# skyepurchase/MeatModeler

Measured on AMD Instinct MI355X. Metric: descriptor-match pairs/sec + BA residuals/sec, 500×1080p frames, 1/2/4/8 GPU, higher is better.
Workload: dtype u8/int32 (match), f64 (BA); 1 GPU; 500 frames 1920x1080, 4000 ORB kpts/frame, BF Hamming 2-NN + ratio, track linking, 2-view DLT, full BA (TRF, Schur, f64 MFMA Cholesky); frames=500, height=1080, width=1920, nfeatures=4000, parallelism=pairs/points x1

## Files before the change

### meatmodeler_amd/csrc/schur.hip

```cpp
#include "ba_eval.h"
#include "chol_init.h"

namespace {

constexpr int SR_WIN = 256;

__global__ __launch_bounds__(256) void point_inverse_kernel(int P, const double *__restrict__ Cd,
                                                            double *__restrict__ Cinv) {
    int p = blockIdx.x * 256 + threadIdx.x;
    if (p >= P) return;
    const double *c = Cd + (size_t)p * 6;
    const double a = c[0], b = c[1], d = c[2], e = c[3], f = c[4], g = c[5];
    const double m00 = e * g - f * f, m01 = d * f - b * g, m02 = b * f - d * e;
    const double det = a * m00 + b * m01 + d * m02;
    const double id = 1.0 / det;
    double *o = Cinv + (size_t)p * 6;
    o[0] = m00 * id;
    o[1] = m01 * id;
    o[2] = m02 * id;
    o[3] = (a * g - d * d) * id;
    o[4] = (b * d - a * f) * id;
    o[5] = (a * e - b * b) * id;
}

__global__ __launch_bounds__(256) void schur_rows_kernel(mm_ba_problem pb, const double *__restrict__ cams,
                                                         const double *__restrict__ pts, const double *__restrict__ Bd,
                                                         const double *__restrict__ Cinv, const double *__restrict__ gc,
                                                         const double *__restrict__ gp, double *__restrict__ S,
                                                         double *__restrict__ v) {
    __shared__ double acc[6][SR_WIN * 6];
    __shared__ double Ks[9];
    __shared__ double cs[6];
    __shared__ double sm[4];
    const int i = blockIdx.x;
    const int w0 = blockIdx.y * SR_WIN;
    const int wn = min(SR_WIN, pb.F - w0);
    const size_t n = (size_t)pb.F * 6;
    for (int e = threadIdx.x; e < 6 * SR_WIN * 6; e += 256) (&acc[0][0])[e] = 0.0;
    if (threadIdx.x < 9) Ks[threadIdx.x] = pb.K[threadIdx.x];
    if (threadIdx.x < 6) cs[threadIdx.x] = cams[(size_t)i * 6 + threadIdx.x];
    __syncthreads();
    double vg[6] = {0, 0, 0, 0, 0, 0};
    for (int e = pb.cam_ptr[i] + threadIdx.x; e < pb.cam_ptr[i + 1]; e += 256) {
        const int o = pb.cam_obs[e];
        const int p = pb.pi[o];
        const double *Xp = pts + (size_t)p * 3;
        Proj pr;
        ba_eval<true, true>(cs, Xp, Ks, pb.obs[2 * (size_t)o], pb.obs[2 * (size_t)o + 1], pr);
        const double *ci = Cinv + (size_t)p * 6;
        const double q00 = ci[0], q01 = ci[1], q02 = ci[2], q11 = ci[3], q12 = ci[4], q22 = ci[5];
        double Y[6][3];
#pragma unroll
        for (int a = 0; a < 6; ++a) {
            const double e0 = pr.Jc[0][a] * pr.Jp[0][0] + pr.Jc[1][a] * pr.Jp[1][0];
            const double e1 = pr.Jc[0][a] * pr.Jp[0][1] + pr.Jc[1][a] * pr.Jp[1][1];
            const double e2 = pr.Jc[0][a] * pr.Jp[0][2] + pr.Jc[1][a] * pr.Jp[1][2];
            Y[a][0] = e0 * q00 + e1 * q01 + e2 * q02;
            Y[a][1] = e0 * q01 + e1 * q11 + e2 * q12;
            Y[a][2] = e0 * q02 + e1 * q12 + e2 * q22;
        }
        if (blockIdx.y == 0) {
            const double g0 = gp[(size_t)p * 3], g1 = gp[(size_t)p * 3 + 1], g2 = gp[(size_t)p * 3 + 2];
#pragma unroll
            for (int a = 0; a < 6; ++a) vg[a] += Y[a][0] * g0 + Y[a][1] * g1 + Y[a][2] * g2;
        }
        for (int e2i = pb.pt_ptr[p]; e2i < pb.pt_ptr[p + 1]; ++e2i) {
            const int o2 = pb.pt_obs[e2i];
            const int f2 = pb.fi[o2];
            if (f2 < w0 || f2 >= w0 + wn) continue;
            Proj p2;
            ba_eval<true, true>(cams + (size_t)f2 * 6, Xp, Ks, pb.obs[2 * (size_t)o2], pb.obs[2 * (size_t)o2 + 1], p2);
            double *dst = &acc[0][(f2 - w0) * 6];
#pragma unroll
            for (int b = 0; b < 6; ++b) {
                const double e0 = p2.Jc[0][b] * p2.Jp[0][0] + p2.Jc[1][b] * p2.Jp[1][0];
                const double e1 = p2.Jc[0][b] * p2.Jp[0][1] + p2.Jc[1][b] * p2.Jp[1][1];
                const double e2 = p2.Jc[0][b] * p2.Jp[0][2] + p2.Jc[1][b] * p2.Jp[1][2];
#pragma unroll
                for (int a = 0; a < 6; ++a)
                    atomicAdd(dst + a * (SR_WIN * 6) + b, Y[a][0] * e0 + Y[a][1] * e1 + Y[a][2] * e2);
            }
        }
    }
    __syncthreads();
    for (int e = threadIdx.x; e < 6 * wn * 6; e += 256) {
        const int a = e / (wn * 6), c = e % (wn * 6);
        const int col = w0 * 6 + c;
        double val = -acc[a][c];
        if (col / 6 == i) val += Bd[(size_t)i * 36 + a * 6 + (col % 6)];
        S[((size_t)i * 6 + a) * n + col] = val;
    }
    if (blockIdx.y == 0) {
#pragma unroll
        for (int a = 0; a < 6; ++a) {
            const double s = block_sum<256>(vg[a], sm);
            if (threadIdx.x == 0) v[(size_t)i * 6 + a] = gc[(size_t)i * 6 + a] - s;
        }
    }
}

#ifndef MM_SP_WAVES
#define MM_SP_WAVES 1
#endif
constexpr int SP_WAVES = MM_SP_WAVES;
constexpr int MAX_SLABS = 64;
struct SlabSync {
    int32_t *ready;
    int32_t *done;
    int32_t seg_count[MAX_SLABS];
    int cams_per_slab;
};
constexpr int CAMTAB = 11;
__device__ __forceinline__ void write_chunk_desc(const mm_ba_problem &pb, int32_t *__restrict__ desc, int64_t first, int64_t stride) {
    for (int64_t k = first; k < pb.n_chunks; k += stride) {
        const int sidx = pb.chunk_seg[k], seg = pb.seg_ids[sidx];
        const int ci = seg / (pb.cam_span + 1), cdd = seg % (pb.cam_span + 1);
        const int c_first = pb.seg_chunk_ptr[sidx];
        int32_t *o = desc + 8 * k;
        o[0] = ci;
        o[1] = ci - cdd;
        o[2] = pb.chunk_begin[k];
        o[3] = pb.chunk_end[k];
        o[4] = sidx;
        o[5] = c_first;
        o[6] = pb.seg_chunk_ptr[sidx + 1] - c_first;
        o[7] = 0;
    }
}
__global__ __launch_bounds__(64) void cam_table_kernel(int F, const double *__restrict__ cams, double *__restrict__ tab,
                                                       int32_t *__restrict__ seg_done, int64_t n_seg, const double *__restrict__ K_lean,
                                                       mm_ba_problem pb, int32_t *__restrict__ desc) {
    const int f = blockIdx.x * 64 + threadIdx.x;
    for (int64_t k = f; k < n_seg; k += (int64_t)gridDim.x * 64) seg_done[k] = 0;
    if (desc) write_chunk_desc(pb, desc, f, (int64_t)gridDim.x * 64);
    if (f >= F) return;
    const double *c = cams + (size_t)f * 6;
    if (K_lean) {
        cam_table2_row(c, K_lean, tab + (size_t)f * CAMTAB2);
        return;
    }
    const CamCoef k = cam_coef_of(c);
    double *t = tab + (size_t)f * CAMTAB;
    for (int q = 0; q < 6; ++q) t[q] = c[q];
    t[6] = k.c;
    t[7] = k.a;
    t[8] = k.b;
    t[9] = k.a1;
    t[10] = k.b1;
}

__device__ __forceinline__ CamVals cam_vals_from_table(const double *__restrict__ t) {
    CamVals v;
    v.rx = uniform_f64(t[0]);
    v.ry = uniform_f64(t[1]);
    v.rz = uniform_f64(t[2]);
    v.tx = uniform_f64(t[3]);
    v.ty = uniform_f64(t[4]);
    v.tz = uniform_f64(t[5]);
    v.k.c = uniform_f64(t[6]);
    v.k.a = uniform_f64(t[7]);
    v.k.b = uniform_f64(t[8]);
    v.k.a1 = uniform_f64(t[9]);
    v.k.b1 = uniform_f64(t[10]);
    return v;
}

constexpr int RED_LD = 65;
__device__ __forceinline__ void wave_lds_barrier() {
    __builtin_amdgcn_fence(__ATOMIC_RELEASE, "wavefront");
    __builtin_amdgcn_wave_barrier();
    __builtin_amdgcn_fence(__ATOMIC_ACQUIRE, "wavefront");
}
__device__ __forceinline__ void wave_reduce_42(const double (&acc)[42], double *slab , int lane, double &out0,
                                               double &out1) {
#pragma unroll
    for (int h = 0; h < 2; ++h) {
#pragma unroll
        for (int q = 0; q < 21; ++q) slab[q * RED_LD + lane] = acc[21 * h + q];
        wave_lds_barrier();
        double s = 0.0;
        if (lane < 21) {
            const double *row = slab + lane * RED_LD;
            double s0 = 0.0, s1 = 0.0, s2 = 0.0, s3 = 0.0;
#pragma unroll
            for (int j = 0; j < 64; j += 4) {
                s0 += row[j];
                s1 += row[j + 1];
                s2 += row[j + 2];
                s3 += row[j + 3];
            }
            s = (s0 + s1) + (s2 + s3);
        }
        if (h == 0)
            out0 = s;
        else
            out1 = s;
        wave_lds_barrier();
    }
}

__global__ __launch_bounds__(64 * SP_WAVES, 2) void schur_pairs_ref_kernel(mm_ba_problem pb, const double *__restrict__ camtab,
                                                                    const double *__restrict__ pts,
                                                                    const double *__restrict__ Cinv,
                                                                    const double *__restrict__ gp,
                                                                    double *partial, const double *__restrict__ Bd,
                                                                    const double *__restrict__ gc, double *S, double *v,
                                                                    int32_t *seg_done, SlabSync slabs, unsigned wg_begin,
                                                                    unsigned wg_total) {
    __shared__ double Ks[9];
    __shared__ double red[SP_WAVES][21 * RED_LD];
    if (threadIdx.x < 9) Ks[threadIdx.x] = pb.K[threadIdx.x];
    __syncthreads();
    const int lane = threadIdx.x & 63;
    const unsigned gpos = blockIdx.x + wg_begin;
    const unsigned wg = (gpos & 1) ? wg_total - 1 - (gpos >> 1) : (gpos >> 1);
    const int64_t c = (int64_t)wg * SP_WAVES + (threadIdx.x >> 6);
    if (c >= pb.n_chunks) return;
    const int sidx = __builtin_amdgcn_readfirstlane(pb.chunk_seg[c]);
    const int seg = __builtin_amdgcn_readfirstlane(pb.seg_ids[sidx]);
    const int i = seg / (pb.cam_span + 1), d = seg % (pb.cam_span + 1);
    const int f2 = i - d;
    const CamVals cv_i = cam_vals_from_table(camtab + (size_t)i * CAMTAB), cv_2 = cam_vals_from_table(camtab + (size_t)f2 * CAMTAB);
    double acc[42];
#pragma unroll
    for (int q = 0; q < 42; ++q) acc[q] = 0.0;
    const int e_end = __builtin_amdgcn_readfirstlane(pb.chunk_end[c]);
    const int e_begin = __builtin_amdgcn_readfirstlane(pb.chunk_begin[c]);
    constexpr int MAXT = 4;
    int oi[MAXT], o2i[MAXT], pidx[MAXT];
#pragma unroll
    for (int k = 0; k < MAXT; ++k) {
        const int e = e_begin + lane + 64 * k;
        const bool in = e < e_end;
        oi[k] = in ? pb.pair_o[e] : -1;
        o2i[k] = in ? pb.pair_o2[e] : -1;
        pidx[k] = in ? (pb.pair_p ? pb.pair_p[e] : -2) : -1;
    }
    auto pair_body = [&](int o, int o2, int p) {
        const double *Xp = pts + (size_t)p * 3;
        Proj pr;
        ba_eval_vals<true, true>(cv_i, Xp, Ks, pb.obs[2 * (size_t)o], pb.obs[2 * (size_t)o + 1], pr);
        const double *ci = Cinv + (size_t)p * 6;
        const double q00 = ci[0], q01 = ci[1], q02 = ci[2], q11 = ci[3], q12 = ci[4], q22 = ci[5];
        double Z[2][3];
#pragma unroll
        for (int m = 0; m < 2; ++m) {
            Z[m][0] = pr.Jp[m][0] * q00 + pr.Jp[m][1] * q01 + pr.Jp[m][2] * q02;
            Z[m][1] = pr.Jp[m][0] * q01 + pr.Jp[m][1] * q11 + pr.Jp[m][2] * q12;
            Z[m][2] = pr.Jp[m][0] * q02 + pr.Jp[m][1] * q12 + pr.Jp[m][2] * q22;
        }
        if (o2 == o) {
            const double g0 = gp[(size_t)p * 3], g1 = gp[(size_t)p * 3 + 1], g2 = gp[(size_t)p * 3 + 2];
            const double z0 = Z[0][0] * g0 + Z[0][1] * g1 + Z[0][2] * g2, z1 = Z[1][0] * g0 + Z[1][1] * g1 + Z[1][2] * g2;
#pragma unroll
            for (int a = 0; a < 6; ++a) acc[36 + a] += pr.Jc[0][a] * z0 + pr.Jc[1][a] * z1;
        }
        Proj p2;
        ba_eval_vals<true, true>(cv_2, Xp, Ks, pb.obs[2 * (size_t)o2], pb.obs[2 * (size_t)o2 + 1], p2);
        double M[2][2];
#pragma unroll
        for (int m = 0; m < 2; ++m)
#pragma unroll
            for (int n_ = 0; n_ < 2; ++n_) M[m][n_] = Z[m][0] * p2.Jp[n_][0] + Z[m][1] * p2.Jp[n_][1] + Z[m][2] * p2.Jp[n_][2];
#pragma unroll
        for (int b = 0; b < 6; ++b) {
            const double t0 = M[0][0] * p2.Jc[0][b] + M[0][1] * p2.Jc[1][b], t1 = M[1][0] * p2.Jc[0][b] + M[1][1] * p2.Jc[1][b];
#pragma unroll
            for (int a = 0; a < 6; ++a) acc[a * 6 + b] += pr.Jc[0][a] * t0 + pr.Jc[1][a] * t1;
        }
    };
    const int trips = (e_end - e_begin + 63) / 64;
    for (int k = 0; k < MAXT; ++k) {
        if (k >= trips) break;
        int o = oi[0], o2 = o2i[0], p = pidx[0];
#pragma unroll
        for (int q = 1; q < MAXT; ++q)
            if (q == k) {
                o = oi[q];
                o2 = o2i[q];
                p = pidx[q];
            }
        if (o >= 0) {
            if (p == -2) p = pb.pi[o];
            pair_body(o, o2, p);
        }
    }
    for (int e = e_begin + lane + 64 * MAXT; e < e_end; e += 64) {
        const int o = pb.pair_o[e], o2 = pb.pair_o2[e];
        pair_body(o, o2, pb.pair_p ? pb.pair_p[e] : pb.pi[o]);
    }
    double tot0, tot1;
    wave_reduce_42(acc, red[threadIdx.x >> 6], lane, tot0, tot1);
    const int c_first = pb.seg_chunk_ptr[sidx], n_ch = pb.seg_chunk_ptr[sidx + 1] - c_first;
    const size_t n = (size_t)pb.F * 6;
    bool writer = true;
    if (n_ch > 1) {
        if (lane < 21) {
            __hip_atomic_store(partial + (size_t)c * 42 + lane, tot0, __ATOMIC_RELAXED, __HIP_MEMORY_SCOPE_AGENT);
            __hip_atomic_store(partial + (size_t)c * 42 + 21 + lane, tot1, __ATOMIC_RELAXED, __HIP_MEMORY_SCOPE_AGENT);
        }
        asm volatile("s_waitcnt vmcnt(0)" ::: "memory");
        __builtin_amdgcn_wave_barrier();
        int last = 0;
        if (lane == 0) last = atomicAdd(seg_done + sidx, 1) == n_ch - 1;
        writer = __shfl(last, 0, 64) != 0;
        if (writer && lane < 21) {
            tot0 = 0.0;
            tot1 = 0.0;
            for (int cc = 0; cc < n_ch; ++cc) {
                tot0 += __hip_atomic_load(partial + (size_t)(c_first + cc) * 42 + lane, __ATOMIC_RELAXED, __HIP_MEMORY_SCOPE_AGENT);
                tot1 += __hip_atomic_load(partial + (size_t)(c_first + cc) * 42 + 21 + lane, __ATOMIC_RELAXED, __HIP_MEMORY_SCOPE_AGENT);
            }
        }
    }
    if (!writer) return;
    if (lane < 21) {
#pragma unroll
        for (int h = 0; h < 2; ++h) {
            const int q = 21 * h + lane;
            const double sum = h == 0 ? tot0 : tot1;
            if (q < 36) {
                double val = -sum;
                if (d == 0) val += Bd[(size_t)i * 36 + q];
                __hip_atomic_store(S + ((size_t)i * 6 + q / 6) * n + (size_t)f2 * 6 + q % 6, val, __ATOMIC_RELAXED, __HIP_MEMORY_SCOPE_AGENT);
                if (d != 0)
                    __hip_atomic_store(S + ((size_t)f2 * 6 + q % 6) * n + (size_t)i * 6 + q / 6, val, __ATOMIC_RELAXED, __HIP_MEMORY_SCOPE_AGENT);
            } else if (d == 0) {
                __hip_atomic_store(v + (size_t)i * 6 + (q - 36), gc[(size_t)i * 6 + (q - 36)] - sum, __ATOMIC_RELAXED, __HIP_MEMORY_SCOPE_AGENT);
            }
        }
    }
    if (slabs.ready) {
        asm volatile("s_waitcnt vmcnt(0)" ::: "memory");
        __builtin_amdgcn_wave_barrier();
        if (lane == 0) {
            const int sl = i / slabs.cams_per_slab;
            if (atomicAdd(slabs.done + sl, 1) == slabs.seg_count[sl] - 1)
                __hip_atomic_store(slabs.ready + sl, 1, __ATOMIC_RELEASE, __HIP_MEMORY_SCOPE_AGENT);
        }
    }
}


struct CamPQ {
    double P[9], q[3];
};
__device__ __forceinline__ double fast_rcp(double x) {
    double y = __builtin_amdgcn_rcp(x);
    double e = fma(-x, y, 1.0);
    y = fma(y, e, y);
    e = fma(-x, y, 1.0);
    return fma(y, e, y);
}

struct LeanJ {
    double Jc[2][6];
    double Jp[2][3];
};
__device__ __forceinline__ void lean_eval(const CamPQ &c, const double *__restrict__ Ks, const double *__restrict__ Jr,
                                          double X0, double X1, double X2, LeanJ &o) {
    const double u0 = fma(c.P[0], X0, fma(c.P[1], X1, fma(c.P[2], X2, c.q[0])));
    const double u1 = fma(c.P[3], X0, fma(c.P[4], X1, fma(c.P[5], X2, c.q[1])));
    const double u2 = fma(c.P[6], X0, fma(c.P[7], X1, fma(c.P[8], X2, c.q[2])));
    const double iz = fast_rcp(u2);
    const double p[2] = {u0 * iz, u1 * iz};
#pragma unroll
    for (int m = 0; m < 2; ++m) {
#pragma unroll
        for (int k = 0; k < 3; ++k) {
            o.Jp[m][k] = fma(-p[m], c.P[6 + k], c.P[3 * m + k]) * iz;
            o.Jc[m][3 + k] = fma(-p[m], Ks[6 + k], Ks[3 * m + k]) * iz;
        }
        const double g0 = X1 * o.Jp[m][2] - X2 * o.Jp[m][1];
        const double g1 = X2 * o.Jp[m][0] - X0 * o.Jp[m][2];
        const double g2 = X0 * o.Jp[m][1] - X1 * o.Jp[m][0];
#pragma unroll
        for (int k = 0; k < 3; ++k) o.Jc[m][k] = fma(g0, Jr[k], fma(g1, Jr[3 + k], g2 * Jr[6 + k]));
    }
}

constexpr int SLAB2 = 32;
struct ChunkDesc {
    int32_t i, f2, e_begin, e_end, sidx, c_first, n_ch, pad;
};
template <bool FORCE>
__device__ __forceinline__ CamPQ cam_pq_scalar(const double *__restrict__ t) {
    CamPQ v;
#pragma unroll
    for (int k = 0; k < 9; ++k) v.P[k] = FORCE ? uniform_f64(t[k]) : t[k];
#pragma unroll
    for (int k = 0; k < 3; ++k) v.q[k] = FORCE ? uniform_f64(t[9 + k]) : t[9 + k];
    return v;
}
template <bool FORCE_UNIFORM>
__device__ __forceinline__ void schur_pairs_body(const mm_ba_problem pb, const double *__restrict__ camtab,
                                                                    const ChunkDesc *__restrict__ desc,
                                                                    const double *__restrict__ pts,
                                                                    const double *__restrict__ Cinv,
                                                                    const double *__restrict__ gp,
                                                                    double *partial, const double *__restrict__ Bd,
                                                                    const double *__restrict__ gc, double *S, double *v,
                                                                    int32_t *seg_done, SlabSync slabs, unsigned wg_begin,
                                                                    unsigned wg_total, const unsigned bx) {
    __shared__ double Ks[9];
    __shared__ double red[SP_WAVES][21 * RED_LD];
    __shared__ double jrs[SP_WAVES][SLAB2];
    if (threadIdx.x < 9) Ks[threadIdx.x] = pb.K[threadIdx.x];
    const int lane = threadIdx.x & 63;
    const int wv = __builtin_amdgcn_readfirstlane((int)(threadIdx.x >> 6));
    const unsigned gpos = bx + wg_begin;
    const unsigned wg = (gpos & 1) ? wg_total - 1 - (gpos >> 1) : (gpos >> 1);
    const int64_t c = (int64_t)wg * SP_WAVES + wv;
    const bool live = c < pb.n_chunks;
    ChunkDesc cd = {};
    if (live) cd = desc[c];
    if (FORCE_UNIFORM) {
        cd.i = __builtin_amdgcn_readfirstlane(cd.i);
        cd.f2 = __builtin_amdgcn_readfirstlane(cd.f2);
        cd.e_begin = __builtin_amdgcn_readfirstlane(cd.e_begin);
        cd.e_end = __builtin_amdgcn_readfirstlane(cd.e_end);
        cd.sidx = __builtin_amdgcn_readfirstlane(cd.sidx);
        cd.c_first = __builtin_amdgcn_readfirstlane(cd.c_first);
        cd.n_ch = __builtin_amdgcn_readfirstlane(cd.n_ch);
    }
    const int i = cd.i, f2 = cd.f2, d = cd.i - cd.f2, sidx = cd.sidx;
    const int e_begin = cd.e_begin, e_end = cd.e_end;
    auto point_of = [&](int e) { return pb.pair_p ? pb.pair_p[e] : pb.pi[pb.pair_o[e]]; };
    auto self_of = [&](int e) { return d == 0 && pb.pair_o[e] == pb.pair_o2[e]; };
    int e = e_begin + lane;
    int p_next = -1;
    bool self_next = false;
    if (live) {
        if (e < e_end) {
            p_next = point_of(e);
            self_next = self_of(e);
        }
        if (lane < 9) jrs[wv][lane] = camtab[(size_t)i * CAMTAB2 + 12 + lane];
        else if (lane >= 16 && lane < 25) jrs[wv][lane] = camtab[(size_t)f2 * CAMTAB2 + 12 + lane - 16];
    }
    __syncthreads();
    if (!live) return;
    const CamPQ cp_i = cam_pq_scalar<FORCE_UNIFORM>(camtab + (size_t)i * CAMTAB2), cp_2 = cam_pq_scalar<FORCE_UNIFORM>(camtab + (size_t)f2 * CAMTAB2);
    const double *Jr_i = jrs[wv], *Jr_2 = jrs[wv] + 16;
    double acc[42];
#pragma unroll
    for (int q = 0; q < 42; ++q) acc[q] = 0.0;
    auto load_xc = [&](int p, double (&x)[12]) {
        if (p >= 0) {
            const double *Xp = pts + (size_t)p * 3, *ci = Cinv + (size_t)p * 6;
            x[0] = Xp[0];
            x[1] = Xp[1];
            x[2] = Xp[2];
#pragma unroll
            for (int q = 0; q < 6; ++q) x[3 + q] = ci[q];
            if (d == 0) {
                x[9] = gp[(size_t)p * 3];
                x[10] = gp[(size_t)p * 3 + 1];
                x[11] = gp[(size_t)p * 3 + 2];
            }
        }
    };
    auto pair_body = [&](int p, bool self, const double (&x)[12]) {
        const double X0 = x[0], X1 = x[1], X2 = x[2];
        const double q00 = x[3], q01 = x[4], q02 = x[5], q11 = x[6], q12 = x[7], q22 = x[8];
        LeanJ a;
        lean_eval(cp_i, Ks, Jr_i, X0, X1, X2, a);
        double Z[2][3];
#pragma unroll
        for (int m = 0; m < 2; ++m) {
            Z[m][0] = a.Jp[m][0] * q00 + a.Jp[m][1] * q01 + a.Jp[m][2] * q02;
            Z[m][1] = a.Jp[m][0] * q01 + a.Jp[m][1] * q11 + a.Jp[m][2] * q12;
            Z[m][2] = a.Jp[m][0] * q02 + a.Jp[m][1] * q12 + a.Jp[m][2] * q22;
        }
        double M[2][2], T[2][6];
        if (d == 0) {
            if (self) {
                const double g0 = x[9], g1 = x[10], g2 = x[11];
                const double z0 = Z[0][0] * g0 + Z[0][1] * g1 + Z[0][2] * g2, z1 = Z[1][0] * g0 + Z[1][1] * g1 + Z[1][2] * g2;
#pragma unroll
                for (int q = 0; q < 6; ++q) acc[36 + q] += a.Jc[0][q] * z0 + a.Jc[1][q] * z1;
            }
#pragma unroll
            for (int m = 0; m < 2; ++m)
#pragma unroll
                for (int n_ = 0; n_ < 2; ++n_) M[m][n_] = Z[m][0] * a.Jp[n_][0] + Z[m][1] * a.Jp[n_][1] + Z[m][2] * a.Jp[n_][2];
#pragma unroll
            for (int b = 0; b < 6; ++b) {
                T[0][b] = M[0][0] * a.Jc[0][b] + M[0][1] * a.Jc[1][b];
                T[1][b] = M[1][0] * a.Jc[0][b] + M[1][1] * a.Jc[1][b];
            }
        } else {
            LeanJ b2;
            lean_eval(cp_2, Ks, Jr_2, X0, X1, X2, b2);
#pragma unroll
            for (int m = 0; m < 2; ++m)
#pragma unroll
                for (int n_ = 0; n_ < 2; ++n_) M[m][n_] = Z[m][0] * b2.Jp[n_][0] + Z[m][1] * b2.Jp[n_][1] + Z[m][2] * b2.Jp[n_][2];
#pragma unroll
            for (int b = 0; b < 6; ++b) {
                T[0][b] = M[0][0] * b2.Jc[0][b] + M[0][1] * b2.Jc[1][b];
                T[1][b] = M[1][0] * b2.Jc[0][b] + M[1][1] * b2.Jc[1][b];
            }
        }
#pragma unroll
        for (int q = 0; q < 6; ++q)
#pragma unroll
            for (int b = 0; b < 6; ++b) acc[q * 6 + b] += a.Jc[0][q] * T[0][b] + a.Jc[1][q] * T[1][b];
    };
    double xc[12];
    load_xc(p_next, xc);
    int p_cur = p_next;
    bool self_cur = self_next;
    {
        const int en = e + 64;
        p_next = en < e_end ? point_of(en) : -1;
        self_next = en < e_end && self_of(en);
    }
#pragma clang loop unroll(disable)
    for (; e - lane < e_end; e += 64) {
        double xn[12];
        load_xc(p_next, xn);
        const int p_nn_e = e + 128;
        const int p_nn = p_nn_e < e_end ? point_of(p_nn_e) : -1;
        const bool self_nn = p_nn_e < e_end && self_of(p_nn_e);
        if (p_cur >= 0) pair_body(p_cur, self_cur, xc);
#pragma unroll
        for (int q = 0; q < 12; ++q) xc[q] = xn[q];
        p_cur = p_next;
        self_cur = self_next;
        p_next = p_nn;
        self_next = self_nn;
    }
    double tot0, tot1;
    wave_reduce_42(acc, red[wv], lane, tot0, tot1);
    const int c_first = cd.c_first, n_ch = cd.n_ch;
    const size_t n = (size_t)pb.F * 6;
    bool writer = true;
    if (n_ch > 1) {
        if (lane < 21) {
            __hip_atomic_store(partial + (size_t)c * 42 + lane, tot0, __ATOMIC_RELAXED, __HIP_MEMORY_SCOPE_AGENT);
            __hip_atomic_store(partial + (size_t)c * 42 + 21 + lane, tot1, __ATOMIC_RELAXED, __HIP_MEMORY_SCOPE_AGENT);
        }
        asm volatile("s_waitcnt vmcnt(0)" ::: "memory");
        __builtin_amdgcn_wave_barrier();
        int last = 0;
        if (lane == 0) last = atomicAdd(seg_done + sidx, 1) == n_ch - 1;
        writer = __shfl(last, 0, 64) != 0;
        if (writer && lane < 21) {
            tot0 = 0.0;
            tot1 = 0.0;
            for (int cc = 0; cc < n_ch; ++cc) {
                tot0 += __hip_atomic_load(partial + (size_t)(c_first + cc) * 42 + lane, __ATOMIC_RELAXED, __HIP_MEMORY_SCOPE_AGENT);
                tot1 += __hip_atomic_load(partial + (size_t)(c_first + cc) * 42 + 21 + lane, __ATOMIC_RELAXED, __HIP_MEMORY_SCOPE_AGENT);
            }
        }
    }
    if (!writer) return;
    const bool through = slabs.ready != nullptr;
    if (lane < 21) {
#pragma unroll
        for (int h = 0; h < 2; ++h) {
            const int q = 21 * h + lane;
            const double sum = h == 0 ? tot0 : tot1;
            if (q < 36) {
                double val = -sum;
                if (d == 0) val += Bd[(size_t)i * 36 + q];
                double *dst = S + ((size_t)i * 6 + q / 6) * n + (size_t)f2 * 6 + q % 6;
                double *mir = S + ((size_t)f2 * 6 + q % 6) * n + (size_t)i * 6 + q / 6;
                if (through) {
                    __hip_atomic_store(dst, val, __ATOMIC_RELAXED, __HIP_MEMORY_SCOPE_AGENT);
                    if (d != 0) __hip_atomic_store(mir, val, __ATOMIC_RELAXED, __HIP_MEMORY_SCOPE_AGENT);
                } else {
                    *dst = val;
                    if (d != 0) *mir = val;
                }
            } else if (d == 0) {
                double *dst = v + (size_t)i * 6 + (q - 36);
                const double val = gc[(size_t)i * 6 + (q - 36)] - sum;
                if (through) __hip_atomic_store(dst, val, __ATOMIC_RELAXED, __HIP_MEMORY_SCOPE_AGENT);
                else *dst = val;
            }
        }
    }
    if (slabs.ready) {
        asm volatile("s_waitcnt vmcnt(0)" ::: "memory");
        __builtin_amdgcn_wave_barrier();
        if (lane == 0) {
            const int sl = i / slabs.cams_per_slab;
            if (atomicAdd(slabs.done + sl, 1) == slabs.seg_count[sl] - 1)
                __hip_atomic_store(slabs.ready + sl, 1, __ATOMIC_RELEASE, __HIP_MEMORY_SCOPE_AGENT);
        }
    }
}
template <int OCC>
__global__ __launch_bounds__(64 * SP_WAVES, OCC) void schur_pairs_kernel(mm_ba_problem pb, const double *__restrict__ camtab,
                                                                    const ChunkDesc *__restrict__ desc,
                                                                    const double *__restrict__ pts,
                                                                    const double *__restrict__ Cinv,
                                                                    const double *__restrict__ gp,
                                                                    double *partial, const double *__restrict__ Bd,
                                                                    const double *__restrict__ gc, double *S, double *v,
                                                                    int32_t *seg_done, SlabSync slabs, unsigned wg_begin,
                                                                    unsigned wg_total) {
    schur_pairs_body<false>(pb, camtab, desc, pts, Cinv, gp, partial, Bd, gc, S, v, seg_done, slabs, wg_begin, wg_total, blockIdx.x);
}
__global__ __launch_bounds__(256) void zero_batch_kernel(const mm_batch_prob *__restrict__ tab, const int32_t *__restrict__ list) {
    const mm_batch_prob &bp = tab[list[blockIdx.y]];
    if (blockIdx.x >= bp.g_zero) return;
    double2 *S2 = reinterpret_cast<double2 *>(bp.S);
    const int64_t n2 = bp.nc * bp.nc / 2;
    for (int64_t i = (int64_t)blockIdx.x * 256 + threadIdx.x; i < n2; i += (int64_t)bp.g_zero * 256) S2[i] = make_double2(0.0, 0.0);
}
__global__ __launch_bounds__(64 * SP_WAVES, 2) void schur_pairs_batch_kernel(const mm_batch_prob *__restrict__ tab, const int32_t *__restrict__ list) {
    const mm_batch_prob &bp = tab[list[blockIdx.y]];
    if (blockIdx.x >= bp.g_pairs) return;
    SlabSync none = {};
    schur_pairs_body<true>(bp.pb, bp.schur_camtab, (const ChunkDesc *)bp.schur_desc, bp.x + bp.nc, bp.Cinv, bp.g + bp.nc, bp.schur_partial, bp.Bd,
                     bp.g, bp.S, bp.v, bp.schur_seg_done, none, 0u, bp.g_pairs, blockIdx.x);
}




__global__ void slab_flag_kernel(int32_t *flags, int s) {
    __hip_atomic_store(flags + s, 1, __ATOMIC_RELEASE, __HIP_MEMORY_SCOPE_AGENT);
}

__global__ void schur_diag_fill_kernel(mm_ba_problem pb, const double *__restrict__ Bd, const double *__restrict__ gc,
                                       double *__restrict__ S, double *__restrict__ v) {
    const int i = blockIdx.x;
    if (pb.cam_ptr[i + 1] != pb.cam_ptr[i]) return;
    const size_t n = (size_t)pb.F * 6;
    if (threadIdx.x < 36) S[((size_t)i * 6 + threadIdx.x / 6) * n + (size_t)i * 6 + threadIdx.x % 6] = Bd[(size_t)i * 36 + threadIdx.x];
    if (threadIdx.x < 6) v[(size_t)i * 6 + threadIdx.x] = gc[(size_t)i * 6 + threadIdx.x];
}

struct PrepExtra {
    mm_damp_spec dmp;
    int zero_bwb;
    int chol_init;
    mm_chol_init_args init;
};
__device__ __forceinline__ void schur_prepare_body(mm_ba_problem pb, const double *__restrict__ cams,
                                                            double *__restrict__ Bd, const double *__restrict__ Cd,
                                                            const double *__restrict__ gc, double *__restrict__ Cinv,
                                                            double *__restrict__ S, double *__restrict__ v,
                                                            double *__restrict__ tab, int32_t *__restrict__ seg_done, bool lean,
                                                            int32_t *__restrict__ desc , const unsigned bx, const unsigned gx,
                                                            const PrepExtra *ex = nullptr) {
    const int b = (int)bx, tid = threadIdx.x;
    for (int64_t k = (int64_t)b * 256 + tid; k < pb.n_seg; k += (int64_t)gx * 256) seg_done[k] = 0;
    if (desc) write_chunk_desc(pb, desc, (int64_t)b * 256 + tid, (int64_t)gx * 256);
    const bool fold = ex && ex->dmp.B;
    double reg = 0.0;
    if (fold) {
        if (ex->dmp.gh2) {
            const double r = trf_damping_value(ex->dmp.gh2[0], ex->dmp.d11[0], ex->dmp.Delta);
            reg = fmax(r, ex->dmp.min_damping);
            if (b == 0 && tid == 0) {
                ex->dmp.damp_out[0] = r;
                ex->dmp.damp_out[1] = reg;
            }
        } else {
            reg = ex->dmp.reg[0];
        }
    }
    if (ex && ex->chol_init) mm_chol_init_body(ex->init, bx, gx);
    const size_t n = (size_t)pb.F * 6;
    if (ex && ex->zero_bwb >= 0) {
        const int nblk = (int)((n + 63) / 64);
        for (size_t r = bx; r < n; r += gx) {
            const int bi = (int)(r >> 6);
            const int lo = bi - ex->zero_bwb < 0 ? 0 : bi - ex->zero_bwb, hi = bi + ex->zero_bwb >= nblk ? nblk - 1 : bi + ex->zero_bwb;
            const size_t c0 = (size_t)lo * 64, c1 = (size_t)(hi + 1) * 64 < n ? (size_t)(hi + 1) * 64 : n;
            const size_t d0 = r / 6 * 6;
            for (size_t c = c0 + 2 * (size_t)tid; c < c1; c += 512)
                if (c < d0 || c >= d0 + 6) *reinterpret_cast<double2 *>(S + r * n + c) = double2{0.0, 0.0};
        }
    }
    const int f = b * 256 + tid;
    if (f < pb.F) {
        const double *c = cams + (size_t)f * 6;
        if (lean) {
            cam_table2_row(c, pb.K, tab + (size_t)f * CAMTAB2);
        } else {
            const CamCoef k = cam_coef_of(c);
            double *t = tab + (size_t)f * CAMTAB;
            for (int q = 0; q < 6; ++q) t[q] = c[q];
            t[6] = k.c;
            t[7] = k.a;
            t[8] = k.b;
            t[9] = k.a1;
            t[10] = k.b1;
        }
    }
    if (b < pb.F) {
        const bool empty = pb.cam_ptr[b + 1] == pb.cam_ptr[b];
        if (tid < 36) {
            double bd;
            if (fold) {
                bd = ex->dmp.B[(size_t)b * 36 + tid];
                if (tid % 7 == 0) {
                    const double s = ex->dmp.si[(size_t)b * 6 + tid / 7];
                    bd = fma(s * s, reg, bd);
                }
                Bd[(size_t)b * 36 + tid] = bd;
            } else {
                bd = Bd[(size_t)b * 36 + tid];
            }
            if (empty)
                S[((size_t)b * 6 + tid / 6) * n + (size_t)b * 6 + tid % 6] = bd;
            else if (ex && ex->zero_bwb >= 0)
                S[((size_t)b * 6 + tid / 6) * n + (size_t)b * 6 + tid % 6] = 0.0;
        }
        if (empty && tid < 6) v[(size_t)b * 6 + tid] = gc[(size_t)b * 6 + tid];
    }
    const int p = b * 256 + tid;
    if (p < pb.P) {
        double a, bq, d, e, ff, g;
        if (fold) {
            const double *c = ex->dmp.C + (size_t)p * 6;
            const double *sp = ex->dmp.si + n + (size_t)p * 3;
            a = fma(sp[0] * sp[0], reg, c[0]);
            bq = c[1];
            d = c[2];
            e = fma(sp[1] * sp[1], reg, c[3]);
            ff = c[4];
            g = fma(sp[2] * sp[2], reg, c[5]);
        } else {
            const double *c = Cd + (size_t)p * 6;
            a = c[0], bq = c[1], d = c[2], e = c[3], ff = c[4], g = c[5];
        }
        const double m00 = e * g - ff * ff, m01 = d * ff - bq * g, m02 = bq * ff - d * e;
        const double det = a * m00 + bq * m01 + d * m02;
        const double id = 1.0 / det;
        double *o = Cinv + (size_t)p * 6;
        o[0] = m00 * id;
        o[1] = m01 * id;
        o[2] = m02 * id;
        o[3] = (a * g - d * d) * id;
        o[4] = (bq * d - a * ff) * id;
        o[5] = (a * e - bq * bq) * id;
    }
}
__global__ __launch_bounds__(256) void schur_prepare_kernel(mm_ba_problem pb, const double *__restrict__ cams,
                                                            double *__restrict__ Bd, const double *__restrict__ Cd,
                                                            const double *__restrict__ gc, double *__restrict__ Cinv,
                                                            double *__restrict__ S, double *__restrict__ v,
                                                            double *__restrict__ tab, int32_t *__restrict__ seg_done, bool lean,
                                                            int32_t *__restrict__ desc) {
    schur_prepare_body(pb, cams, Bd, Cd, gc, Cinv, S, v, tab, seg_done, lean, desc, blockIdx.x, gridDim.x);
}
__global__ __launch_bounds__(256) void schur_prepare_damped_kernel(mm_ba_problem pb, const double *__restrict__ cams,
                                                                   double *__restrict__ Bd, const double *__restrict__ gc,
                                                                   double *__restrict__ Cinv, double *__restrict__ S,
                                                                   double *__restrict__ v, double *__restrict__ tab,
                                                                   int32_t *__restrict__ seg_done, int32_t *__restrict__ desc,
                                                                   PrepExtra ex) {
    schur_prepare_body(pb, cams, Bd, nullptr, gc, Cinv, S, v, tab, seg_done, true, desc, blockIdx.x, gridDim.x, &ex);
}
__global__ __launch_bounds__(256) void schur_prepare_batch_kernel(const mm_batch_prob *__restrict__ tab, const int32_t *__restrict__ list) {
    const mm_batch_prob &bp = tab[list[blockIdx.y]];
    if (blockIdx.x >= bp.g_prep) return;
    schur_prepare_body(bp.pb, bp.x, bp.Bd, bp.Cd, bp.g, bp.Cinv, bp.S, bp.v, bp.schur_camtab, bp.schur_seg_done, true, bp.schur_desc,
                       blockIdx.x, bp.g_prep);
}


__global__ __launch_bounds__(256) void pairs_count_kernel(mm_ba_problem pb, int32_t *__restrict__ cnt,
                                                          int32_t *__restrict__ span_out) {
    const int64_t o = (int64_t)blockIdx.x * 256 + threadIdx.x;
    int dmax = 0;
    if (o < pb.O) {
        const int f = pb.fi[o], p = pb.pi[o];
        int c = 0;
        for (int e = pb.pt_ptr[p]; e < pb.pt_ptr[p + 1]; ++e) {
            const int d = f - pb.fi[pb.pt_obs[e]];
            c += d >= 0;
            dmax = max(dmax, d);
        }
        cnt[o] = c;
    }
    for (int off = 32; off > 0; off >>= 1) dmax = max(dmax, __shfl_down(dmax, off, 64));
    if ((threadIdx.x & 63) == 0 && dmax > __hip_atomic_load(span_out, __ATOMIC_RELAXED, __HIP_MEMORY_SCOPE_AGENT)) atomicMax(span_out, dmax);
}

__global__ __launch_bounds__(256) void pairs_emit_kernel(mm_ba_problem pb, const int64_t *__restrict__ offsets, int span,
                                                         int32_t *__restrict__ key, int32_t *__restrict__ po,
                                                         int32_t *__restrict__ po2) {
    const int64_t o = (int64_t)blockIdx.x * 256 + threadIdx.x;
    if (o >= pb.O) return;
    const int f = pb.fi[o], p = pb.pi[o];
    int64_t w = offsets[o];
    for (int e = pb.pt_ptr[p]; e < pb.pt_ptr[p + 1]; ++e) {
        const int o2 = pb.pt_obs[e];
        const int d = f - pb.fi[o2];
        if (d < 0) continue;
        key[w] = f * (span + 1) + d;
        po[w] = (int32_t)o;
        po2[w] = o2;
        ++w;
    }
}

}

extern "C" int mm_ba_pairs_count(mm_ctx *ctx, const mm_ba_problem *pb, int32_t *cnt, int32_t *span_out) {
    if (!ctx) return MM_ERR_ARG;
    if (!pb || !cnt || !span_out || (pb->O > 0 && (!pb->fi || !pb->pi || !pb->pt_ptr || !pb->pt_obs)))
        return mm_fail(ctx, MM_ERR_ARG, "mm_ba_pairs_count: bad argument");
    MM_HIP(ctx, hipMemsetAsync(span_out, 0, sizeof(int32_t), ctx->stream));
    if (pb->O == 0) return MM_OK;
    MM_LAUNCH(ctx, "pairs_count_kernel", pairs_count_kernel, dim3((unsigned)((pb->O + 255) / 256)), dim3(256), 0, *pb, cnt,
              span_out);
    return MM_OK;
}

extern "C" int mm_ba_pairs_emit(mm_ctx *ctx, const mm_ba_problem *pb, const int64_t *offsets, int span, int32_t *key,
                                int32_t *pair_o, int32_t *pair_o2) {
    if (!ctx) return MM_ERR_ARG;
    if (!pb || !offsets || !key || !pair_o || !pair_o2 || span < 0) return mm_fail(ctx, MM_ERR_ARG, "mm_ba_pairs_emit: bad argument");
    if (pb->O == 0) return MM_OK;
    if ((int64_t)pb->F * (span + 1) > 0x7fffffffLL) return mm_fail(ctx, MM_ERR_ARG, "mm_ba_pairs_emit: F * (span + 1) overflows the key");
    MM_LAUNCH(ctx, "pairs_emit_kernel", pairs_emit_kernel, dim3((unsigned)((pb->O + 255) / 256)), dim3(256), 0, *pb, offsets,
              span, key, pair_o, pair_o2);
    return MM_OK;
}

extern "C" size_t mm_ba_schur_workspace_bytes(const mm_ba_problem *pb) {
    if (!pb || pb->n_chunks <= 0) return 0;
    return mm_align_up((size_t)pb->n_chunks * 42 * sizeof(double), 256)  +
           mm_align_up((size_t)pb->n_seg * sizeof(int32_t), 256)  +
           mm_align_up(2 * MAX_SLABS * sizeof(int32_t), 256)  +
           mm_align_up((size_t)pb->F * CAMTAB2 * sizeof(double), 256)  +
// ... 211 lines not shown
```

Measured before the change: 9112 billion descriptor pairs/s (match stage).

## Restructure Schur pair loop into templated software pipeline with clamped indices

Rewrites the per-chunk Schur-complement accumulation loop as a templated routine specialised on diagonal vs off-diagonal blocks and on whether a direct pair-to-point index exists. Index loads are clamped instead of predicated, and the loop rotates a ring of register buffers with a configurable prefetch depth, with an optional second level of index indirection prefetched ahead. The goal is to hide gather latency and remove per-iteration branches and copies. The cost is more register pressure from the extra buffers and more code from the four instantiations. The metric shown is the match stage, which this kernel does not touch.

```diff
diff --git a/meatmodeler_amd/csrc/schur.hip b/meatmodeler_amd/csrc/schur.hip
--- a/meatmodeler_amd/csrc/schur.hip
+++ b/meatmodeler_amd/csrc/schur.hip
@@ -1,5 +1,6 @@
 #include "ba_eval.h"
 #include "chol_init.h"
+#include <type_traits>
 
 namespace {
 
@@ -103,6 +104,11 @@
 #define MM_SP_WAVES 1
 #endif
 constexpr int SP_WAVES = MM_SP_WAVES;
+#ifndef MM_SP_DEPTH
+#define MM_SP_DEPTH 1
+#endif
+constexpr int SP_DEPTH = MM_SP_DEPTH;
+static_assert(SP_DEPTH == 1 || SP_DEPTH == 2, "MM_SP_DEPTH: one or two trips ahead");
 constexpr int MAX_SLABS = 64;
 struct SlabSync {
     int32_t *ready;
@@ -425,15 +431,15 @@
     }
     const int i = cd.i, f2 = cd.f2, d = cd.i - cd.f2, sidx = cd.sidx;
     const int e_begin = cd.e_begin, e_end = cd.e_end;
-    auto point_of = [&](int e) { return pb.pair_p ? pb.pair_p[e] : pb.pi[pb.pair_o[e]]; };
-    auto self_of = [&](int e) { return d == 0 && pb.pair_o[e] == pb.pair_o2[e]; };
-    int e = e_begin + lane;
-    int p_next = -1;
-    bool self_next = false;
+    const int e_last = e_end - 1;
+    const bool any = live && e_end > e_begin;
+    int p0 = 0, o0 = 0, o0b = 0;
     if (live) {
-        if (e < e_end) {
-            p_next = point_of(e);
-            self_next = self_of(e);
+        if (any) {
+            const int ec = min(e_begin + lane, e_last);
+            if (!pb.pair_p || d == 0) o0 = pb.pair_o[ec];
+            if (d == 0) o0b = pb.pair_o2[ec];
+            p0 = pb.pair_p ? pb.pair_p[ec] : pb.pi[o0];
         }
         if (lane < 9) jrs[wv][lane] = camtab[(size_t)i * CAMTAB2 + 12 + lane];
         else if (lane >= 16 && lane < 25) jrs[wv][lane] = camtab[(size_t)f2 * CAMTAB2 + 12 + lane - 16];
@@ -445,91 +451,117 @@
     double acc[42];
 #pragma unroll
     for (int q = 0; q < 42; ++q) acc[q] = 0.0;
-    auto load_xc = [&](int p, double (&x)[12]) {
-        if (p >= 0) {
+    auto run_trips = [&](auto diag_c, auto hasp_c) {
+        constexpr bool DIAG = decltype(diag_c)::value, HAS_P = decltype(hasp_c)::value;
+        constexpr int NX = DIAG ? 12 : 9;
+        constexpr int NB = SP_DEPTH + 1;
+        auto gather = [&](int p, double (&x)[NX]) {
             const double *Xp = pts + (size_t)p * 3, *ci = Cinv + (size_t)p * 6;
             x[0] = Xp[0];
             x[1] = Xp[1];
             x[2] = Xp[2];
 #pragma unroll
             for (int q = 0; q < 6; ++q) x[3 + q] = ci[q];
-            if (d == 0) {
+            if (DIAG) {
                 x[9] = gp[(size_t)p * 3];
                 x[10] = gp[(size_t)p * 3 + 1];
                 x[11] = gp[(size_t)p * 3 + 2];
             }
+        };
+        auto pair_body = [&](bool self, const double (&x)[NX]) {
+            const double X0 = x[0], X1 = x[1], X2 = x[2];
+            const double q00 = x[3], q01 = x[4], q02 = x[5], q11 = x[6], q12 = x[7], q22 = x[8];
+            LeanJ a;
+            lean_eval(cp_i, Ks, Jr_i, X0, X1, X2, a);
+            double Z[2][3];
+#pragma unroll
+            for (int m = 0; m < 2; ++m) {
+                Z[m][0] = a.Jp[m][0] * q00 + a.Jp[m][1] * q01 + a.Jp[m][2] * q02;
+                Z[m][1] = a.Jp[m][0] * q01 + a.Jp[m][1] * q11 + a.Jp[m][2] * q12;
+                Z[m][2] = a.Jp[m][0] * q02 + a.Jp[m][1] * q12 + a.Jp[m][2] * q22;
+            }
+            double M[2][2], T[2][6];
+            if (DIAG) {
+                if (self) {
+                    const double g0 = x[NX - 3], g1 = x[NX - 2], g2 = x[NX - 1];
+                    const double z0 = Z[0][0] * g0 + Z[0][1] * g1 + Z[0][2] * g2, z1 = Z[1][0] * g0 + Z[1][1] * g1 + Z[1][2] * g2;
+#pragma unroll
+                    for (int q = 0; q < 6; ++q) acc[36 + q] += a.Jc[0][q] * z0 + a.Jc[1][q] * z1;
+                }
+#pragma unroll
+                for (int m = 0; m < 2; ++m)
+#pragma unroll
+                    for (int n_ = 0; n_ < 2; ++n_) M[m][n_] = Z[m][0] * a.Jp[n_][0] + Z[m][1] * a.Jp[n_][1] + Z[m][2] * a.Jp[n_][2];
+#pragma unroll
+                for (int b = 0; b < 6; ++b) {
+                    T[0][b] = M[0][0] * a.Jc[0][b] + M[0][1] * a.Jc[1][b];
+                    T[1][b] = M[1][0] * a.Jc[0][b] + M[1][1] * a.Jc[1][b];
+                }
+            } else {
+                LeanJ b2;
+                lean_eval(cp_2, Ks, Jr_2, X0, X1, X2, b2);
+#pragma unroll
+                for (int m = 0; m < 2; ++m)
+#pragma unroll
+                    for (int n_ = 0; n_ < 2; ++n_) M[m][n_] = Z[m][0] * b2.Jp[n_][0] + Z[m][1] * b2.Jp[n_][1] + Z[m][2] * b2.Jp[n_][2];
+#pragma unroll
+                for (int b = 0; b < 6; ++b) {
+                    T[0][b] = M[0][0] * b2.Jc[0][b] + M[0][1] * b2.Jc[1][b];
+                    T[1][b] = M[1][0] * b2.Jc[0][b] + M[1][1] * b2.Jc[1][b];
+                }
+            }
+#pragma unroll
+            for (int q = 0; q < 6; ++q)
+#pragma unroll
+                for (int b = 0; b < 6; ++b) acc[q * 6 + b] += a.Jc[0][q] * T[0][b] + a.Jc[1][q] * T[1][b];
+        };
+        auto pair_at = [&](int eb, int k) { return min(eb + lane + 64 * k, e_last); };
+        constexpr int LEAD = SP_DEPTH + (HAS_P ? 0 : 1);
+        double X[NB][NX];
+        bool selfq[NB];
+#pragma unroll
+        for (int k = 0; k < NB; ++k) selfq[k] = HAS_P && k == NB - 1 && o0 == o0b;
+        int p1 = p0;
+        int o2r = o0;
+        __builtin_amdgcn_s_waitcnt(0x0F70);
+        auto trip = [&](int eb, const double (&xc)[NX], double (&xn)[NX]) {
+            const int e2 = pair_at(eb, NB);
+            int idx2, o3 = 0, sa = 0, sb = 0;
+            if (HAS_P) {
+                idx2 = pb.pair_p[e2];
+            } else {
+                o3 = pb.pair_o[pair_at(eb, NB + 1)];
+                idx2 = pb.pi[o2r];
+            }
+            if (DIAG) {
+                sa = HAS_P ? pb.pair_o[e2] : o2r;
+                sb = pb.pair_o2[e2];
+            }
+            gather(p1, xn);
+            if ((unsigned)(eb + lane - e_begin) < (unsigned)(e_end - e_begin)) pair_body(selfq[0], xc);
+            p1 = idx2;
+            o2r = o3;
+#pragma unroll
+            for (int k = 0; k + 1 < NB; ++k) selfq[k] = selfq[k + 1];
+            selfq[NB - 1] = sa == sb;
+        };
+#pragma clang loop unroll(disable)
+        for (int eb = e_begin - 64 * LEAD; eb < e_end;) {
+#pragma unroll
+            for (int j = 0; j < NB; ++j) {
+                trip(eb, X[j], X[(j + SP_DEPTH) % NB]);
+                eb += 64;
+            }
         }
     };
-    auto pair_body = [&](int p, bool self, const double (&x)[12]) {
-        const double X0 = x[0], X1 = x[1], X2 = x[2];
-        const double q00 = x[3], q01 = x[4], q02 = x[5], q11 = x[6], q12 = x[7], q22 = x[8];
-        LeanJ a;
-        lean_eval(cp_i, Ks, Jr_i, X0, X1, X2, a);
-        double Z[2][3];
-#pragma unroll
-        for (int m = 0; m < 2; ++m) {
-            Z[m][0] = a.Jp[m][0] * q00 + a.Jp[m][1] * q01 + a.Jp[m][2] * q02;
-            Z[m][1] = a.Jp[m][0] * q01 + a.Jp[m][1] * q11 + a.Jp[m][2] * q12;
-            Z[m][2] = a.Jp[m][0] * q02 + a.Jp[m][1] * q12 + a.Jp[m][2] * q22;
-        }
-        double M[2][2], T[2][6];
+    if (any) {
         if (d == 0) {
-            if (self) {
-                const double g0 = x[9], g1 = x[10], g2 = x[11];
-                const double z0 = Z[0][0] * g0 + Z[0][1] * g1 + Z[0][2] * g2, z1 = Z[1][0] * g0 + Z[1][1] * g1 + Z[1][2] * g2;
-#pragma unroll
-                for (int q = 0; q < 6; ++q) acc[36 + q] += a.Jc[0][q] * z0 + a.Jc[1][q] * z1;
-            }
-#pragma unroll
-            for (int m = 0; m < 2; ++m)
-#pragma unroll
-                for (int n_ = 0; n_ < 2; ++n_) M[m][n_] = Z[m][0] * a.Jp[n_][0] + Z[m][1] * a.Jp[n_][1] + Z[m][2] * a.Jp[n_][2];
-#pragma unroll
-            for (int b = 0; b < 6; ++b) {
-                T[0][b] = M[0][0] * a.Jc[0][b] + M[0][1] * a.Jc[1][b];
-                T[1][b] = M[1][0] * a.Jc[0][b] + M[1][1] * a.Jc[1][b];
-            }
+            if (pb.pair_p) run_trips(std::true_type{}, std::true_type{});
+            else run_trips(std::true_type{}, std::false_type{});
         } else {
-            LeanJ b2;
-            lean_eval(cp_2, Ks, Jr_2, X0, X1, X2, b2);
-#pragma unroll
-            for (int m = 0; m < 2; ++m)
-#pragma unroll
-                for (int n_ = 0; n_ < 2; ++n_) M[m][n_] = Z[m][0] * b2.Jp[n_][0] + Z[m][1] * b2.Jp[n_][1] + Z[m][2] * b2.Jp[n_][2];
-#pragma unroll
-            for (int b = 0; b < 6; ++b) {
-                T[0][b] = M[0][0] * b2.Jc[0][b] + M[0][1] * b2.Jc[1][b];
-                T[1][b] = M[1][0] * b2.Jc[0][b] + M[1][1] * b2.Jc[1][b];
-            }
-        }
-#pragma unroll
-        for (int q = 0; q < 6; ++q)
-#pragma unroll
-            for (int b = 0; b < 6; ++b) acc[q * 6 + b] += a.Jc[0][q] * T[0][b] + a.Jc[1][q] * T[1][b];
-    };
-    double xc[12];
-    load_xc(p_next, xc);
-    int p_cur = p_next;
-    bool self_cur = self_next;
-    {
-        const int en = e + 64;
-        p_next = en < e_end ? point_of(en) : -1;
-        self_next = en < e_end && self_of(en);
-    }
-#pragma clang loop unroll(disable)
-    for (; e - lane < e_end; e += 64) {
-        double xn[12];
-        load_xc(p_next, xn);
-        const int p_nn_e = e + 128;
-        const int p_nn = p_nn_e < e_end ? point_of(p_nn_e) : -1;
-        const bool self_nn = p_nn_e < e_end && self_of(p_nn_e);
-        if (p_cur >= 0) pair_body(p_cur, self_cur, xc);
-#pragma unroll
-        for (int q = 0; q < 12; ++q) xc[q] = xn[q];
-        p_cur = p_next;
-        self_cur = self_next;
-        p_next = p_nn;
-        self_next = self_nn;
+            if (pb.pair_p) run_trips(std::false_type{}, std::true_type{});
+            else run_trips(std::false_type{}, std::false_type{});
+        }
     }
     double tot0, tot1;
     wave_reduce_42(acc, red[wv], lane, tot0, tot1);
```

After: 9160 billion descriptor pairs/s (match stage), median of 4. No clear change (+0.5%).
